# truemeat001/Simple-Raytracing-Render

Hardware: AMD Instinct MI355X
Metric: Msamples/s (rays x bounces) + HBM GB/s vs roofline, Cornell+teapot 1024spp (higher is better)
Workload: dtype f32

## Files before the change

simple-raytracing-render_amd/csrc/kernels.h:

```cpp
#pragma once
#include <hip/hip_runtime.h>

#include <cstdint>

#include "device_scene.h"

namespace srr {

struct SceneView {
  const DObj* objs;
  int n_world;
  int has_media;
  const DXform* xforms;
  const DSphere* spheres;
  const DRect* rects;
  const DStandaloneTri* stris;
  const DMesh* meshes;
  const float4* nodes;
  const float4* node4;
  int node4_lds;
  int node4_total;
  const float4* node4q;
  int node4_lds_q;
  int use_q;
// ... 60 lines not shown
  uint32_t l = 0;
  while ((1ull << l) < d) ++l;
  const uint32_t p = 31 + l;
  return UDiv31{(uint32_t)(((1ull << p) + d - 1) / d), p};
}

struct PathWork {
  const int32_t* pixels;
  const double* sobol;
  int npix, spp_w;
  int s_base;
  int nx, ny;
  UDiv31 div_spp, div_nx;
  uint64_t base_seed;
  int64_t n_paths;
  int max_depth;
  unsigned long long* cursor;
  unsigned long long* counters;
  float* sample;
  float* raw;
  uint8_t* rays;
  int keep_spp, keep_s0;
  float4* rec;
  int lanes;
  int* err;
  int stack_cap;
  int2* gstack;
  int gstack_cap;
  unsigned long long* wave_times;
  int deep_tries;
  float* slow_rays;
  unsigned* slow_count;
  int walk_q;
};

enum PathsCtr : int {
  kCtrWorldRays = 0,
  kCtrCursor = 1,
  kCtrError = 2,
  kCtrTicksRefill = 4,
  kCtrTicksWorld,
  kCtrTicksMesh,
  kCtrTicksShade,
  kCtrTicksFold,
  kCtrWaveIters = 9,
  kCtrTicksRecord = 10,
  kCtrStackOverflows = 11,
  kCtrDeepTraversals = 12,
  kCtrTicksMixture = 13,
  kCtrMixtureRounds = 14,
  kCtrMixtureCapped = 15,
  kCtrTicksBeck = 16, kCtrTicksSpec, kCtrTicksDiffSetup,
  kCtrItsBeck, kCtrItsSpec, kCtrItsDiff,
  kCtrLanesBeck, kCtrLanesSpec, kCtrLanesDiff,
  kCtrLanesInPath,
  kCtrMeshSteps, kCtrMeshLaneSteps, kCtrMeshWalkers,
  kCtrLeafTicks, kCtrLeafPasses,
  kCtrStepFetch, kCtrStepSlab, kCtrStepOrder,
  kCtrBeckAttempts,
  kCtrBeckAttemptsMax,
  kCtrSuspended = 36,
  kCtrTicksCamOnly = 37, kCtrItsCamOnly,
  kCtrTicksPretrace = 39, kCtrPretracePasses, kCtrShadeRounds,
  kPathsCtrCount
};
constexpr int kPathsCtrWords = 48;
static_assert(kPathsCtrCount == 42 && kPathsCtrCount <= kPathsCtrWords, "PathsCtr fits FrameSlot::ctr");
static_assert(kCtrTicksFold == kCtrTicksRefill + 4 && kCtrTicksFold < kCtrWaveIters, "phase ticks");
static_assert(kCtrTicksDiffSetup == kCtrTicksBeck + 2 && kCtrItsBeck == kCtrTicksBeck + 3 && kCtrItsDiff == kCtrItsBeck + 2 &&
                  kCtrLanesBeck == kCtrItsBeck + 3 && kCtrLanesDiff == kCtrLanesBeck + 2 && kCtrLanesInPath == 25,
              "family words");
static_assert(kCtrMeshSteps == 26 && kCtrStepOrder == kCtrStepFetch + 2 && kCtrBeckAttemptsMax == 35 &&
                  kCtrBeckAttemptsMax < kCtrSuspended, "mesh words");
static_assert(kCtrDeepTraversals == kCtrStackOverflows + 1, "TraceCtx::ovf counts overflows, ovf[1] deep traversals");
static_assert(kCtrItsCamOnly == 38 && kCtrShadeRounds == 41, "camera-only and pre-trace words");
#ifndef SRR_KSTACK
#define SRR_KSTACK 8
#endif
constexpr int kPathsLdsStack = SRR_KSTACK;
constexpr int kPathsGlobalStack = 56;

constexpr int kPathsWorldLdsBytes = 8192;
#ifndef SRR_LDS_NODES
#define SRR_LDS_NODES 96
#endif
constexpr int kPathsLdsNodes = SRR_LDS_NODES;

constexpr int kRingRayWords = 11;
constexpr int kRingHitWord = kRingRayWords;
constexpr int kRingWordsHit = kRingHitWord + 3;
constexpr int ring_words(bool pretrace) { return pretrace ? kRingWordsHit : kRingRayWords; }
static_assert(ring_words(false) == 11 && ring_words(true) == 14 && kRingHitWord + 2 < kRingWordsHit, "ring entry layout");

constexpr int kLdsPerCu = 160 * 1024;
constexpr int paths_lds_fixed(int bs, bool wl) {
  return (wl ? kPathsWorldLdsBytes : 16) + 8 * kPathsLdsStack * bs + bs;
}
constexpr int paths_lds_nodes_big(bool pretrace) {
  return (kLdsPerCu - paths_lds_fixed(1024, true) - 4 * ring_words(pretrace) * 1024) / 128;
}
// ... 118 lines not shown
```

simple-raytracing-render_amd/csrc/kernels.hip:

```cpp
#include <hip/hip_runtime.h>

#include <cfloat>
#include <algorithm>
#include <cstdint>
#include <cstdlib>
#include <cstring>

#include "device_scene.h"
#include "devmath.h"
#include "kernels.h"
#include "../../include/srr/merl.h"

namespace srr {
namespace dev {

SRR_D V3 sphere_center(const DSphere& s, float tm, bool moving) {
  V3 c0 = v3(s.c0[0], s.c0[1], s.c0[2]);
  if (!moving) return c0;
  V3 c1 = v3(s.c1[0], s.c1[1], s.c1[2]);
  return c0 + ((tm - s.t0) / (s.t1 - s.t0)) * (c1 - c0);
}

SRR_D bool sphere_hit(const DSphere& s, bool moving, const Ray& r, float tmin, float tmax, float& t) {
  V3 oc = r.o - sphere_center(s, r.tm, moving);
// ... 2562 lines not shown
  float tm;
  double sx, sy;
  sobol2_point((uint32_t)(W.s_base + (int)s), sx, sy);
  camera_ray(S, pix, W.s_base + s, sx, sy, W.nx, W.ny, W.base_seed, o, d, tm, rng, &W.div_nx);
  r = Ray{o, d, tm};
}

template <int BS>
SRR_D void ring_put(lds_ptr<float> e, const Ray& r, const Rng& rng) {
  e[0] = r.o.x;
  e[BS] = r.o.y;
  e[2 * BS] = r.o.z;
  e[3 * BS] = r.d.x;
  e[4 * BS] = r.d.y;
  e[5 * BS] = r.d.z;
  e[6 * BS] = r.tm;
  e[7 * BS] = __uint_as_float((uint32_t)rng.lcg);
  e[8 * BS] = __uint_as_float((uint32_t)(rng.lcg >> 32));
  e[9 * BS] = __uint_as_float((uint32_t)rng.pcg);
  e[10 * BS] = __uint_as_float((uint32_t)(rng.pcg >> 32));
}

template <int BS>
SRR_D void ring_get_ray(lds_ptr<const float> e, Ray& r) {
  r = Ray{v3(e[0], e[BS], e[2 * BS]), v3(e[3 * BS], e[4 * BS], e[5 * BS]), e[6 * BS]};
}
template <int BS>
SRR_D void ring_get(lds_ptr<const float> e, Ray& r, Rng& rng) {
  ring_get_ray<BS>(e, r);
  rng.lcg = (uint64_t)__float_as_uint(e[7 * BS]) | ((uint64_t)__float_as_uint(e[8 * BS]) << 32);
  rng.pcg = (uint64_t)__float_as_uint(e[9 * BS]) | ((uint64_t)__float_as_uint(e[10 * BS]) << 32);
}

constexpr int kNoHit = -2;
template <int BS>
SRR_D void ring_put_hit(lds_ptr<float> e, int obj, int prim, float t) {
  e[kRingHitWord * BS] = __int_as_float(obj);
  e[(kRingHitWord + 1) * BS] = __int_as_float(prim);
  e[(kRingHitWord + 2) * BS] = t;
}
template <int BS>
SRR_D WorldHit ring_get_hit(lds_ptr<const float> e) {
  return WorldHit{__float_as_int(e[kRingHitWord * BS]), __float_as_int(e[(kRingHitWord + 1) * BS]), e[(kRingHitWord + 2) * BS]};
}

template <int BS, bool HIT>
SRR_D void ring_fill(lds_ptr<float> ring, const SceneView& S, const PathWork& W, uint32_t nb, uint32_t n_paths) {
  const uint32_t gi = nb + (uint32_t)lane_id();
  if (gi < n_paths) {
    Ray gr;
    Rng grng;
    path_camera_ray(S, W, gi, gr, grng);
    ring_put<BS>(ring + lane_id(), gr, grng);
    if (HIT) ring_put_hit<BS>(ring + lane_id(), kNoHit, -1, 0.f);
  }
}

template <int BS, bool HIT>
SRR_D void ring_take(lds_ptr<const float> e, Ray& r, Rng& rng, WorldHit& w) {
  ring_get<BS>(e, r, rng);
  if (HIT) w = ring_get_hit<BS>(e);
}

struct PathsArgs {
  SceneView S;
  PathWork W;
};
#if defined(__HIP_DEVICE_COMPILE__)
template <class T>
using kptr = const __attribute__((address_space(4))) T*;
SRR_D kptr<PathsArgs> paths_args() {
  kptr<PathsArgs> p = (kptr<PathsArgs>)__builtin_amdgcn_kernarg_segment_ptr();
  asm volatile("" : "+s"(p));
  return p;
}
#else
SRR_D const PathsArgs* paths_args() { return nullptr; }
#endif

struct PoolRanks {
  uint32_t cnt;
  uint32_t rank;
  uint32_t avail;
};
SRR_D PoolRanks pool_ranks(uint64_t nm, uint32_t pool, uint32_t pool_end) {
  return PoolRanks{(uint32_t)__popcll(nm), (uint32_t)__popcll(nm & ((1ull << lane_id()) - 1)), pool_end - pool};
}
SRR_D uint32_t pool_arm(uint32_t nxt_lane0) {
  if (lane_id() == 0) nxt_lane0 = (uint32_t)atomicAdd(paths_args()->W.cursor, (unsigned long long)kPoolChunk);
  return nxt_lane0;
}

#ifdef SRR_SLOW_RAYS
SRR_D void slow_ray_record(const PathWork& W, int g, int depth, const Ray& r_in, uint64_t t_w0, int steps, const WorldHit& wh,
                           int slot) {
// ... 14 lines not shown
      e[13] = wh.t;
      e[14] = __int_as_float(slot);
      e[15] = __int_as_float((int)(t_w0 & 0x7fffffff));
    }
  }
}
#endif

constexpr int kTpWords = 8, kTfWords = kCtrBeckAttemptsMax - kCtrTicksBeck + 1, kTzWords = 2, kTptWords = 3;
constexpr int kTpPhases = kCtrTicksFold - kCtrTicksRefill + 1;
template <int Q>
constexpr int tp_at() {
  constexpr int at = Q >= kCtrTicksRefill && Q <= kCtrTicksFold ? Q - kCtrTicksRefill
                     : Q == kCtrTicksRecord ? kTpPhases : Q == kCtrTicksMixture ? kTpPhases + 1
                     : Q == kCtrMixtureRounds ? kTpPhases + 2 : -1;
  static_assert(at >= 0 && at < kTpWords, "not a word of tp");
  return at;
}
template <int Q>
constexpr int tf_at() {
  static_assert(Q >= kCtrTicksBeck && Q <= kCtrBeckAttemptsMax, "not a word of tf");
  return Q - kCtrTicksBeck;
}
template <int Q>
constexpr int tz_at() {
  static_assert(Q >= kCtrTicksCamOnly && Q < kCtrTicksCamOnly + kTzWords, "not a word of tz");
  return Q - kCtrTicksCamOnly;
}
template <int Q>
constexpr int tpt_at() {
  static_assert(Q >= kCtrTicksPretrace && Q < kCtrTicksPretrace + kTptWords, "not a word of tpt");
  return Q - kCtrTicksPretrace;
}

template <bool MEDIA, bool ALLFAM, int MINB, bool TIMED = false, bool WL = true, bool QUAD = false, bool CQ = false,
          int BS = kPathsBlock, bool SP = false>
#ifdef SRR_NUM_VGPR
#define SRR_PATHS_VGPR_ATTR __attribute__((amdgpu_num_vgpr(SRR_NUM_VGPR)))
#else
#define SRR_PATHS_VGPR_ATTR
#endif
__global__ void __launch_bounds__(BS, MINB) SRR_PATHS_VGPR_ATTR k_paths(PathsArgs A) {
  static_assert(BS == kPathsBlock || BS == 1024, "block size");
  (void)A;
  uint64_t tp[kTpWords] = {0, 0, 0, 0, 0, 0, 0, 0};
  uint64_t tf[kTfWords] = {0, 0, 0, 0, 0, 0, 0, 0, 0, 0, 0, 0, 0, 0, 0, 0, 0, 0, 0, 0};
  uint64_t tz[kTzWords] = {0, 0};
  uint64_t it = 0;
  uint64_t tpt[kTptWords] = {0, 0, 0};
  constexpr int TR = TR_BVH4_PRUNE | (WL ? TR_WL : 0) | (QUAD ? TR_QUAD : 0) | (CQ ? TR_Q : 0) | (BS == 1024 ? TR_BIG : 0) |
                     ((SP && !QUAD && !CQ) ? TR_SUSP : 0);
  __shared__ uint4 s_world[WL ? kWorldLdsBytes / 16 : 1];
  const auto view = [&]() {
    SceneView S = paths_args()->S;
    if constexpr (WL) {
      const char* b = (const char*)s_world;
      S.objs = (const DObj*)(b + S.world_off[0]);
      S.xforms = (const DXform*)(b + S.world_off[1]);
      S.spheres = (const DSphere*)(b + S.world_off[2]);
      S.rects = (const DRect*)(b + S.world_off[3]);
      S.stris = (const DStandaloneTri*)(b + S.world_off[4]);
      S.meshes = (const DMesh*)(b + S.world_off[5]);
      S.media = (const DMedium*)(b + S.world_off[6]);
      S.mats = (const DMat*)(b + S.world_off[7]);
      S.texs = (const DTex*)(b + S.world_off[8]);
      S.lights = (const DLight*)(b + S.world_off[9]);
// ... 18 lines not shown
  const uint32_t n_paths = (uint32_t)paths_args()->W.n_paths;
  const uint64_t t_start = paths_args()->W.wave_times ? __builtin_amdgcn_s_memrealtime() : 0;
  {
    const SceneView S0 = paths_args()->S;
    if constexpr (WL)
      for (int i = threadIdx.x; i < S0.world_words; i += blockDim.x) s_world[i] = S0.world_blob[i];
    const int n_lds_nodes = lds_nodes(S0);
    if (CQ)
      for (int i = threadIdx.x; i < n_lds_nodes * 4; i += blockDim.x) s_n4[i] = S0.node4q[i];
    else
      for (int i = threadIdx.x; i < n_lds_nodes * 8; i += blockDim.x) s_n4[i] = S0.node4[i];
  }
  __syncthreads();
  const int slot = blockIdx.x * blockDim.x + threadIdx.x;
  const auto rec_at = [&](const PathWork& W, int k) -> float4* {
    int s = slot;
    asm volatile("" : "+v"(s));
    return W.rec + ((size_t)k * W.lanes + s);
  };
  int g = -1;
  uint32_t pool = 0, pool_end = 0;
  uint32_t nxt_lane0 = 0;
  bool nxt_armed = false;
  uint32_t nxt_base = 0;
  bool nxt_ready = false;
  Ray r{};
  Rng rng{};
  int depth = 0;
  int walking = 0;
  uint32_t nrays = 0;
  uint32_t n_events = 0;
  constexpr uint32_t kCapped = 1, kSuspended = 1u << 12;
  uint32_t n_iter = 0, max_rounds = 0;
  WorldHit w{kNoHit, -1, 0};
  bool fill = false;
  for (;;) {
    ++n_iter;
    uint64_t tq = TIMED ? __builtin_amdgcn_s_memtime() : 0;
    if constexpr (!PT) {
    w = WorldHit{-1, -1, 0};
    const bool need = g < 0;
    const uint64_t nm = __ballot(need);
    if (nm && pool < n_paths) {
      const SceneView S = view();
      const PathWork W = work();
      const PoolRanks k = pool_ranks(nm, pool, pool_end);
      const uint32_t cnt = k.cnt, rank = k.rank, avail = k.avail;
      uint32_t idx = 0;
      if (RING) {
        if (need && rank < avail) {
          const uint32_t i0 = pool + rank;
          if (i0 < n_paths) {
            g = (int)i0;
            ring_take<BS, false>(ringw + (i0 - ring_base), r, rng, w);
            depth = 0;
          }
        }
        if (avail >= cnt) {
          pool += cnt;
        } else {
          uint32_t nb;
          if (nxt_armed) {
            nb = nxt_ready ? nxt_base : __builtin_amdgcn_readfirstlane(nxt_lane0);
            nxt_armed = false;
            nxt_ready = false;
          } else {
            uint32_t b = 0;
            if (lane_id() == 0) b = (uint32_t)atomicAdd(W.cursor, (unsigned long long)kPoolChunk);
            nb = __builtin_amdgcn_readfirstlane(b);
          }
          ring_fill<BS, false>(ringw, S, W, nb, n_paths);
          __builtin_amdgcn_fence(__ATOMIC_SEQ_CST, "wavefront");
          ring_base = nb;
          if (need && rank >= avail) {
            const uint32_t i1 = nb + (rank - avail);
            if (i1 < n_paths) {
              g = (int)i1;
              ring_take<BS, false>(ringw + (i1 - nb), r, rng, w);
              depth = 0;
            }
          }
          pool = nb + (cnt - avail);
          pool_end = nb + (uint32_t)kPoolChunk;
        }
      } else if (avail >= cnt) {
        idx = pool + rank;
        pool += cnt;
      } else {
        uint32_t nb;
        if (nxt_armed) {
          nb = nxt_ready ? nxt_base : __builtin_amdgcn_readfirstlane(nxt_lane0);
          nxt_armed = false;
          nxt_ready = false;
        } else {
          uint32_t b = 0;
          if (lane_id() == 0) b = (uint32_t)atomicAdd(W.cursor, (unsigned long long)kPoolChunk);
          nb = __builtin_amdgcn_readfirstlane(b);
        }
        idx = rank < avail ? pool + rank : nb + (rank - avail);
        pool = nb + (cnt - avail);
        pool_end = nb + (uint32_t)kPoolChunk;
      }
      if (!RING && need && idx < n_paths) {
        g = (int)idx;
        path_camera_ray(S, W, idx, r, rng);
        depth = 0;
      }
    }
    if (!nxt_armed && pool_end < n_paths) {
      nxt_lane0 = pool_arm(nxt_lane0);
      nxt_armed = true;
    }
    if (__ballot(g >= 0) == 0) break;
    if (TIMED) tf[tf_at<kCtrLanesInPath>()] += __popcll(__ballot(g >= 0));
    if (TIMED) {
      __builtin_amdgcn_s_waitcnt(0);
      const uint64_t t = __builtin_amdgcn_s_memtime();
      tp[tp_at<kCtrTicksRefill>()] += t - tq;
      tq = t;
      ++it;
    }
    }
    const bool fill_now = PT && fill;
    bool act = g >= 0 && (!PT || w.obj == kNoHit);
    Ray tr = r;
    if constexpr (PT) {
      if (fill_now) {
        act = ring_base + (uint32_t)lane_id() < n_paths && !walking;
        if (act) ring_get_ray<BS>(ringw + lane_id(), tr);
      }
      if (TIMED) {
        tf[tf_at<kCtrLanesInPath>()] += __popcll(__ballot(g >= 0));
        ++it;
      }
    }
    if (act) {
      const SceneView S = view();
      const PathWork W = work();
      TraceCtx cx{nullptr, to_lds(s_node + threadIdx.x), to_lds(s_t + threadIdx.x)};
      cx.lds_nodes = (const __attribute__((address_space(3))) f32x4*)to_lds(s_n4);
      cx.lds_count = lds_nodes(S);
      cx.st_cap = min(W.stack_cap, kStack);
      cx.ovf = W.counters + kCtrStackOverflows;
      cx.gst = W.gstack;
      cx.gst_cap = W.gstack ? W.gstack_cap : 0;
      cx.gst_stride = W.lanes;
      cx.slot = slot;
      if constexpr ((TR & TR_SUSP) != 0) {
        cx.walk_thr = vreg(fill_now ? 0 : (int)((__popcll(__ballot(true)) * (uint32_t)paths_args()->W.walk_q) >> 6));
        cx.resume = fill_now ? vreg(0) : walking;
        cx.susp = vreg(0);
      }
#ifdef SRR_SLOW_RAYS
      const uint64_t t_w0 = __builtin_amdgcn_s_memrealtime();
      cx.last_steps = 0;
      const Ray r_in = tr;
#endif
      const WorldHit wh =
          world_hit<MEDIA, TIMED ? (TR_BVH4_TIMED | (WL ? TR_WL : 0) | (SP ? TR_SUSP : 0)) : TR>(S, tr, rng, cx);
      if (fill_now) {
        ring_put_hit<BS>(ringw + lane_id(), wh.obj, wh.prim, wh.t);
      } else {
        w = wh;
        if constexpr ((TR & TR_SUSP) != 0) {
          walking = cx.susp;
          if (walking) {
            w.obj = PT ? kNoHit : -1;
            n_events += kSuspended;
          }
        }
      }
#ifdef SRR_SLOW_RAYS
      slow_ray_record(W, g, depth, r_in, t_w0, cx.last_steps, wh, slot);
#endif
      if (TIMED) {
        const uint64_t t = __builtin_amdgcn_s_memtime();
        if (fill_now) {
          tpt[tpt_at<kCtrTicksPretrace>()] += t - tq;
          ++tpt[tpt_at<kCtrPretracePasses>()];
        } else {
          if (__ballot(depth != 0) == 0) {
            tz[tz_at<kCtrTicksCamOnly>()] += t - tq;
            ++tz[tz_at<kCtrItsCamOnly>()];
          }
          tp[tp_at<kCtrTicksWorld>()] += t - tq - cx.mesh_cycles;
          tp[tp_at<kCtrTicksMesh>()] += cx.mesh_cycles;
          tf[tf_at<kCtrMeshSteps>()] += cx.mesh_steps;
          tf[tf_at<kCtrMeshLaneSteps>()] += cx.mesh_lane_steps;
          tf[tf_at<kCtrMeshWalkers>()] += cx.mesh_walkers;
          tf[tf_at<kCtrLeafTicks>()] += cx.leaf_cycles;
          tf[tf_at<kCtrLeafPasses>()] += cx.leaf_passes;
          tf[tf_at<kCtrStepFetch>()] += cx.step_parts[0];
          tf[tf_at<kCtrStepSlab>()] += cx.step_parts[1];
          tf[tf_at<kCtrStepOrder>()] += cx.step_parts[2];
        }
        tq = t;
      }
    }
    if constexpr (PT) {
      if (fill_now) {
        __builtin_amdgcn_fence(__ATOMIC_SEQ_CST, "wavefront");
        fill = false;
      }
    }
    if (nxt_armed && !nxt_ready) {
      nxt_base = __builtin_amdgcn_readfirstlane(nxt_lane0);
      nxt_ready = true;
    }
#pragma nounroll
    for (int round = 0; round < (PT ? 2 : 1); ++round) {
    if constexpr (PT) {
      if (TIMED) tq = __builtin_amdgcn_s_memtime();
      const bool need = g < 0;
      const uint64_t nm = __ballot(need);
      if (nm && pool < n_paths) {
        const PoolRanks k = pool_ranks(nm, pool, pool_end);
        const uint32_t cnt = k.cnt, rank = k.rank, avail = k.avail;
        if (need && rank < avail) {
          const uint32_t i0 = pool + rank;
          if (i0 < n_paths) {
            g = (int)i0;
            ring_take<BS, true>(ringw + (i0 - ring_base), r, rng, w);
            depth = 0;
          }
        }
        if (avail >= cnt) {
          pool += cnt;
        } else {
          const SceneView S = view();
          const PathWork W = work();
          uint32_t nb;
          if (nxt_armed) {
            nb = nxt_ready ? nxt_base : __builtin_amdgcn_readfirstlane(nxt_lane0);
            nxt_armed = false;
            nxt_ready = false;
          } else {
            uint32_t b = 0;
            if (lane_id() == 0) b = (uint32_t)atomicAdd(W.cursor, (unsigned long long)kPoolChunk);
            nb = __builtin_amdgcn_readfirstlane(b);
          }
          __builtin_amdgcn_fence(__ATOMIC_SEQ_CST, "wavefront");
          ring_fill<BS, true>(ringw, S, W, nb, n_paths);
          __builtin_amdgcn_fence(__ATOMIC_SEQ_CST, "wavefront");
          ring_base = nb;
          pool = nb;
          pool_end = nb + (uint32_t)kPoolChunk;
          fill = nb < n_paths;
        }
      }
      if (TIMED) {
        __builtin_amdgcn_s_waitcnt(0);
        const uint64_t t = __builtin_amdgcn_s_memtime();
        tp[tp_at<kCtrTicksRefill>()] += t - tq;
        tq = t;
      }
      if (fill) break;
    }
    const bool sh = g >= 0 && (!PT || w.obj != kNoHit);
    if constexpr (PT) {
      if (__ballot(sh) == 0) break;
      if (TIMED) ++tpt[tpt_at<kCtrShadeRounds>()];
    }
    bool done = sh && (PT || !walking);
    V3 C = v3(0.f);
    bool diff = false, pend = false;
    int natt = 0;
    uint64_t fam_dt[3] = {0, 0, 0};
    DiffSetup ds{};
    V3 d_atten = v3(0.f), d_n = v3(0.f), d_dir = v3(0.f);
    float d_pdf = 0;
    int d_tries = 0;
    bool d_dead = false;
    if (sh) {
      if (w.obj >= 0) {
        const SceneView S = view();
        const PathWork W = work();
        const HitRec h = world_record<TR>(S, r, w);
        const int kind = h.mat >= 0 ? S.mats[h.mat].kind : -1;
        if (TIMED) {
          __builtin_amdgcn_s_waitcnt(0);
          const uint64_t t = __builtin_amdgcn_s_memtime();
          tp[tp_at<kCtrTicksRecord>()] += t - tq;
          tq = t;
        }
        const int fam = family_of(h.mat, kind, depth, W.max_depth);
        if (TIMED) {
          const uint64_t mb = __ballot(fam == FAM_BECK), ms = __ballot(fam == FAM_SPEC),
                         md = __ballot(fam == FAM_DIFF && S.n_lights > 0);
          tf[tf_at<kCtrItsBeck>()] += mb != 0; tf[tf_at<kCtrItsSpec>()] += ms != 0; tf[tf_at<kCtrItsDiff>()] += md != 0;
          tf[tf_at<kCtrLanesBeck>()] += __popcll(mb); tf[tf_at<kCtrLanesSpec>()] += __popcll(ms); tf[tf_at<kCtrLanesDiff>()] += __popcll(md);
        }
        if (fam == FAM_TERM) {
          C = hit_emitted(S, h.mat, r.d, h.p, h.n, h.u, h.v);
        } else if ((!ALLFAM || fam == FAM_DIFF) && S.n_lights > 0) {
          const DMat M = S.mats[h.mat];
          d_atten = tex_value(S, M.tex, h.u, h.v, h.p);
          Bsdf f;
          f.kind = M.kind;
          f.n = h.n;
          f.uvw = onb_from_w(h.n);
          f.A = M.p[0];
          f.B = M.p[1];
          bsdf_prepare<false>(f, r.d);
          ds = diff_setup(f, h.p);
          d_dead = bsdf_dead(S, f, h.p);
          (void)drand(rng);
          d_n = h.n;
          diff = pend = true;
          done = false;
          if (TIMED) fam_dt[2] = __builtin_amdgcn_s_memtime() - tq;
        } else {
          const DMat M = S.mats[h.mat];
          float4 rec;
          bool sp;
          V3 nd;
          float nt;
          const uint64_t tb = TIMED ? __builtin_amdgcn_s_memtime() : 0;
          if (!ALLFAM || fam == FAM_DIFF) scatter<FAM_DIFF>(S, M, r.d, r.tm, h.p, h.n, h.u, h.v, rng, rec, sp, nd, nt);
          else if (fam == FAM_BECK) {
            scatter<FAM_BECK>(S, M, r.d, r.tm, h.p, h.n, h.u, h.v, rng, rec, sp, nd, nt, TIMED ? &natt : nullptr);
            if (TIMED) fam_dt[0] = __builtin_amdgcn_s_memtime() - tb;
          } else {
            scatter<FAM_SPEC>(S, M, r.d, r.tm, h.p, h.n, h.u, h.v, rng, rec, sp, nd, nt);
            if (TIMED) fam_dt[1] = __builtin_amdgcn_s_memtime() - tb;
          }
          if (depth >= W.max_depth || slot >= W.lanes) atomicOr(W.err, 2);
          else *rec_at(W, depth) = rec;
          if (!sp && S.n_lights > 0 && rec.w == 0) n_events += kCapped;
          r = Ray{h.p, nd, nt};
          ++depth;
          done = false;
        }
      }
    }
    if (TIMED) {
      int sum = natt, mx = natt;
      for (int o = 32; o > 0; o >>= 1) {
        sum += __shfl_xor(sum, o);
        mx = max(mx, __shfl_xor(mx, o));
      }
      tf[tf_at<kCtrBeckAttempts>()] += sum;
      tf[tf_at<kCtrBeckAttemptsMax>()] += mx;
      for (int q = 0; q < 3; ++q) {
        uint64_t m = fam_dt[q];
        for (int o = 32; o > 0; o >>= 1) m = max(m, (uint64_t)__shfl_xor((unsigned long long)m, o));
        tf[tf_at<kCtrTicksBeck>() + q] += m;
      }
    }
    if (__ballot(pend)) {
      const SceneView S = view();
      const uint64_t t_mix = TIMED ? __builtin_amdgcn_s_memtime() : 0;
      int rounds = skip_mixture(S, ds, d_dead, pend, d_tries, rng.lcg, d_dir, d_pdf, 1);
      if (__ballot(pend)) rounds += coop_mixture(S, ds, pend, d_tries, rng.lcg, d_dir, d_pdf, paths_args()->W.deep_tries);
      if (TIMED) {
        tp[tp_at<kCtrTicksMixture>()] += __builtin_amdgcn_s_memtime() - t_mix;
        tp[tp_at<kCtrMixtureRounds>()] += rounds;
      }
      max_rounds = max(max_rounds, (uint32_t)rounds);
    }
    if (diff) {
      const PathWork W = work();
      if (d_pdf == 0) n_events += kCapped;
      float c = dot(d_n, unit_vector(d_dir));
      if (c < 0) c = 0;
      const V3 as = d_atten * (c / kPi);
      if (depth >= W.max_depth || slot >= W.lanes) atomicOr(W.err, 2);
      else *rec_at(W, depth) = make_float4(as.x, as.y, as.z, d_pdf);
      r = Ray{ds.p, d_dir, r.tm};
      ++depth;
    }
    if (sh) {
      const PathWork W = work();
      if (PT) w.obj = kNoHit;
      if (TIMED) {
        const uint64_t t = __builtin_amdgcn_s_memtime();
        tp[tp_at<kCtrTicksShade>()] += t - tq;
        tq = t;
      }
      if (done && (g >= W.n_paths || depth > W.max_depth)) {
        atomicOr(W.err, 4);
        g = -1;
        done = false;
      }
      if (done) {
        int k = depth - 1;
        for (; k >= 0; k -= 4) {
          float4 a[4];
#pragma unroll
          for (int j = 0; j < 4; ++j) a[j] = k - j >= 0 ? rec_load(rec_at(W, k - j)) : make_float4(0, 0, 0, 0);
#pragma unroll
          for (int j = 0; j < 4; ++j) {
            if (k - j < 0) break;
            const V3 av = v3(a[j].x, a[j].y, a[j].z);
            if (__float_as_uint(a[j].w) == kSpecMark) C = av * C;
            else C = v3(0.f) + (av * C) / a[j].w;
          }
        }
        if (W.raw) {
          const size_t kq = (size_t)(g / W.spp_w) * W.keep_spp + W.keep_s0 + (size_t)(g % W.spp_w);
          W.raw[3 * kq] = C.x;
          W.raw[3 * kq + 1] = C.y;
          W.raw[3 * kq + 2] = C.z;
          W.rays[kq] = (uint8_t)(depth + 1);
        }
        if (!(C.x == C.x)) C.x = 0;
        if (!(C.y == C.y)) C.y = 0;
        if (!(C.z == C.z)) C.z = 0;
        nts(&W.sample[3 * (size_t)g], C.x);
        nts(&W.sample[3 * (size_t)g + 1], C.y);
        nts(&W.sample[3 * (size_t)g + 2], C.z);
        nrays += depth + 1;
        g = -1;
      }
      if (TIMED) tp[tp_at<kCtrTicksFold>()] += __builtin_amdgcn_s_memtime() - tq;
    }
    }
    if constexpr (PT) {
      if (!nxt_armed && pool_end < n_paths) {
        nxt_lane0 = pool_arm(nxt_lane0);
        nxt_armed = true;
      }
      if (!fill && pool >= n_paths && __ballot(g >= 0) == 0) break;
    }
  }
  const PathWork W = work();
  if (TIMED && lane_id() == 0) {
    for (int q = 0; q < kTpPhases; ++q) atomicAdd(W.counters + kCtrTicksRefill + q, (unsigned long long)tp[q]);
    atomicAdd(W.counters + kCtrWaveIters, (unsigned long long)it);
    atomicAdd(W.counters + kCtrTicksRecord, (unsigned long long)tp[tp_at<kCtrTicksRecord>()]);
    atomicAdd(W.counters + kCtrTicksMixture, (unsigned long long)tp[tp_at<kCtrTicksMixture>()]);
    atomicAdd(W.counters + kCtrMixtureRounds, (unsigned long long)tp[tp_at<kCtrMixtureRounds>()]);
    for (int q = 0; q < kTfWords; ++q) atomicAdd(W.counters + kCtrTicksBeck + q, (unsigned long long)tf[q]);
    for (int q = 0; q < kTzWords; ++q) atomicAdd(W.counters + kCtrTicksCamOnly + q, (unsigned long long)tz[q]);
    for (int q = 0; q < kTptWords; ++q) atomicAdd(W.counters + kCtrTicksPretrace + q, (unsigned long long)tpt[q]);
  }

  unsigned long long tot = nrays;
  for (int o = 32; o > 0; o >>= 1) tot += __shfl_xor(tot, o);
  if (lane_id() == 0 && tot) atomicAdd(W.counters + kCtrWorldRays, tot);
  if (__ballot(n_events != 0)) {
    unsigned long long cap = n_events & (kSuspended - 1), su = n_events / kSuspended;
    for (int o = 32; o > 0; o >>= 1) {
      cap += __shfl_xor(cap, o);
      su += __shfl_xor(su, o);
    }
    if (lane_id() == 0) {
      if (cap) atomicAdd(W.counters + kCtrMixtureCapped, cap);
      if (su) atomicAdd(W.counters + kCtrSuspended, su);
    }
  }
  if (W.wave_times && lane_id() == 0) {
    const size_t wv = (size_t)(blockIdx.x * blockDim.x + threadIdx.x) / 64;
    W.wave_times[4 * wv] = t_start;
    W.wave_times[4 * wv + 1] = __builtin_amdgcn_s_memrealtime();
    W.wave_times[4 * wv + 2] = tot;
    W.wave_times[4 * wv + 3] = n_iter | ((unsigned long long)max_rounds << 32);
  }
}

constexpr int kAccChunk = 16;
struct AccOut {
  float* out;
  int scale_ns;
};
SRR_D void acc_write(float* acc, AccOut o, size_t a, float cx, float cy, float cz) {
  acc[a] = cx;
  acc[a + 1] = cy;
// ... 1026 lines not shown
```

simple-raytracing-render_amd/csrc/renderer.cpp:

```cpp
#include "renderer.h"

#include "multi.h"

#include <algorithm>
#include <chrono>
#include <cstdlib>
#include <cstring>
#include <memory>
#include <thread>
#include <cstdio>

namespace srr {

constexpr int kVisitWords = 3 + 2 * 64;

#define RCHK(x)                                                        \
  do {                                                                 \
    hipError_t e_ = (x);                                               \
    if (e_ != hipSuccess) {                                            \
      err = std::string(#x) + ": " + hipGetErrorString(e_);            \
      return SRR_EIO;                                                  \
    }                                                                  \
  } while (0)

// ... 311 lines not shown
  RCHK(hipEventCreate(&F.ev_end));
  RCHK(hipMalloc((void**)&F.ctr, kPathsCtrWords * sizeof(unsigned long long)));
  RCHK(hipHostMalloc((void**)&F.ctr_host, kPathsCtrWords * sizeof(unsigned long long)));
  return 0;
}

void slot_free(FrameSlot& F) {
  (void)hipFree(F.rec);
  (void)hipFree(F.gstack);
  (void)hipFree(F.sample);
  (void)hipFree(F.ctr);
  (void)hipFree(F.acc);
  if (F.ctr_host) (void)hipHostFree(F.ctr_host);
  for (hipEvent_t e : F.win_ev) (void)hipEventDestroy(e);
  if (F.ev_beg) (void)hipEventDestroy(F.ev_beg);
  if (F.ev_end) (void)hipEventDestroy(F.ev_end);
  if (F.own_stream && F.st) (void)hipStreamDestroy(F.st);
  F = FrameSlot{};
}

static void release_window(FrameSlot& F) {
  if (!F.sample) return;
  (void)hipFree(F.sample);
  F.sample = nullptr;
  F.sample_cap = 0;
}

struct PathsSetup {
  int gst_cap = 0;
  int walk_q = 0;
  int deep_tries = 32;
  int stack_cap = kPathsLdsStack;
  size_t budget = 0;
};

static int paths_prepare(srr_renderer* r, FrameSlot& F, int max_depth, PathsSetup& ps, std::string& err) {
  if (!r->pw_lanes) r->pw_lanes = paths_lanes_per_device(r->view, r->device);
  const size_t rec_need = (size_t)r->pw_lanes * std::max(1, max_depth);
  if (rec_need > F.rec_cap) {
    (void)hipFree(F.rec);
    F.rec = nullptr;
    F.rec_cap = 0;
    RCHK(hipMalloc((void**)&F.rec, rec_need * sizeof(float4)));
    F.rec_cap = rec_need;
  }
  const char* gs_env = getenv("SRR_GSTACK");
  ps.gst_cap = (r->has_meshes && !(gs_env && !atoi(gs_env))) ? kPathsGlobalStack : 0;
  if (ps.gst_cap && !F.gstack)
    RCHK(hipMalloc((void**)&F.gstack, (size_t)ps.gst_cap * r->pw_lanes * sizeof(int2) + 3 * (size_t)r->pw_lanes * sizeof(float4)));
  const char* wq_env = getenv("SRR_WALK_Q");
  ps.walk_q = wq_env ? std::max(0, std::min(64, atoi(wq_env))) : r->walk_q_default;
  ps.budget = (size_t)16384 << 20;
  if (const char* e = getenv("SRR_WINDOW_MB")) ps.budget = (size_t)std::max(1, atoi(e)) << 20;
  ps.budget /= (size_t)std::max(1, r->window_share);
  const char* dt_env = getenv("SRR_DEEP_TRIES");
  ps.deep_tries = dt_env ? std::max(0, atoi(dt_env)) : 32;
  ps.stack_cap = kPathsLdsStack;
  if (const char* e = getenv("SRR_STACK_CAP")) ps.stack_cap = std::max(1, std::min(kPathsLdsStack, atoi(e)));
  return 0;
}

static int window_samples(const PathsSetup& ps, int64_t npix, int spp) {
  const int64_t w_max = std::max<int64_t>(1, (((int64_t)1 << 31) - 1) / std::max<int64_t>(1, npix));
  int W = (int)std::max<int64_t>(
      1, std::min<int64_t>(std::min<int64_t>(spp, w_max), (int64_t)(ps.budget / (12 * (size_t)npix))));
  if (W < spp && W >= 16) W &= ~3;
  return W;
}

static int ensure_window(srr_renderer* r, FrameSlot& F, size_t win_paths, std::string& err) {
  if (win_paths > F.sample_cap) {
    (void)hipFree(F.sample);
    F.sample = nullptr;
    F.sample_cap = 0;
    hipError_t e = hipMalloc((void**)&F.sample, win_paths * 3 * sizeof(float));
    if (e == hipErrorOutOfMemory) {
      (void)hipGetLastError();
      if (&F == &r->sync_slot) {
        drain_async(r);
        for (FrameSlot& A : r->async_slots) release_window(A);
      } else {
        release_window(r->sync_slot);
      }
      e = hipMalloc((void**)&F.sample, win_paths * 3 * sizeof(float));
    }
    RCHK(e);
    F.sample_cap = win_paths;
  }
  return 0;
}

static PathWork paths_work(srr_renderer* r, FrameSlot& F, const srr_params* p, const PathsSetup& ps,
                           const int32_t* pixels, int64_t npix, int s_first, int Wn) {
  PathWork w{};
  w.pixels = pixels;
  w.sobol = r->sobol + 2 * (size_t)s_first;
  w.npix = (int)npix;
  w.spp_w = Wn;
  w.s_base = s_first;
  w.nx = p->nx;
  w.ny = p->ny;
  w.div_spp = make_udiv31((uint32_t)Wn);
  w.div_nx = make_udiv31((uint32_t)p->nx);
  w.base_seed = p->base_seed;
  w.n_paths = (int64_t)npix * Wn;
  w.max_depth = p->max_depth;
  w.cursor = F.ctr + kCtrCursor;
  w.counters = F.ctr;
  w.sample = F.sample;
  w.rec = F.rec;
  w.err = (int*)(F.ctr + kCtrError);
  const int64_t bl = paths_block_lanes(r->view);
  w.lanes = (int)std::min<int64_t>(r->pw_lanes, ((w.n_paths + bl - 1) / bl) * bl);
  w.stack_cap = ps.stack_cap;
  w.gstack = ps.gst_cap ? F.gstack : nullptr;
  w.gstack_cap = ps.gst_cap;
  w.deep_tries = ps.deep_tries;
  w.walk_q = ps.gst_cap ? ps.walk_q : 0;
  return w;
}

static int paths_enqueue(srr_renderer* r, FrameSlot& F, const srr_params* p, bool identity, int64_t npix,
                         float* acc, bool zero_pending, int64_t acc_total, float* d_mean, bool diagnostics,
                         std::string& err) {
  const bool keep = (p->flags & SRR_FLAG_KEEP_PATHS) != 0;
  hipStream_t st = F.st;
  PathsSetup ps;
  {
    const int rc = paths_prepare(r, F, p->max_depth, ps, err);
    if (rc < 0) return rc;
  }
  const int W = window_samples(ps, npix, p->spp);
  if ((int64_t)npix * W >= ((int64_t)1 << 31)) {
    err = "frame too large for one sample window (npix >= 2^31)";
    return SRR_EINVAL;
  }
  {
    const int rc = ensure_window(r, F, (size_t)npix * W, err);
    if (rc < 0) return rc;
  }
  RCHK(hipMemsetAsync(F.ctr, 0, kPathsCtrWords * sizeof(unsigned long long), st));
  const bool want_sums = (p->flags & SRR_FLAG_SUMS) != 0;
  const int n_windows = (p->spp + W - 1) / W;
  while ((int)F.win_ev.size() < 2 * n_windows) {
    hipEvent_t e;
    RCHK(hipEventCreate(&e));
    F.win_ev.push_back(e);
  }
  F.n_windows = n_windows;
  const bool all_fam = !r->diffuse_only;
  static const bool want_wave_times = getenv("SRR_WAVE_TIMES") != nullptr;
// ... 88 lines not shown
  if (getenv("SRR_PATHS_TIMING") && ctr[kCtrWaveIters]) {
    const double it = (double)ctr[kCtrWaveIters];
    fprintf(stderr, "k_paths per wave-iteration (ticks): refill %.0f  world %.0f  mesh %.0f  record %.0f  scatter %.0f  fold %.0f  (%llu wave-iterations)\n",
            ctr[kCtrTicksRefill] / it, ctr[kCtrTicksWorld] / it, ctr[kCtrTicksMesh] / it, ctr[kCtrTicksRecord] / it,
            (ctr[kCtrTicksShade] - ctr[kCtrTicksRecord]) / it, ctr[kCtrTicksFold] / it, ctr[kCtrWaveIters]);
    fprintf(stderr, "  scatter: mixture loop %.0f ticks, %.2f rounds per wave-iteration\n", ctr[kCtrTicksMixture] / it,
            ctr[kCtrMixtureRounds] / it);
    auto per = [](unsigned long long a, unsigned long long b) { return b ? (double)a / (double)b : 0.0; };
    fprintf(stderr, "  families: beck %.0f ticks/it (runs in %.1f %% of its, %.1f lanes/run), spec %.0f (%.1f %%, %.1f), "
                    "diff set-up %.0f (%.1f %%, %.1f); lanes in a path %.1f of 64\n",
            ctr[kCtrTicksBeck] / it, 100 * ctr[kCtrItsBeck] / it, per(ctr[kCtrLanesBeck], ctr[kCtrItsBeck]),
            ctr[kCtrTicksSpec] / it, 100 * ctr[kCtrItsSpec] / it, per(ctr[kCtrLanesSpec], ctr[kCtrItsSpec]),
            ctr[kCtrTicksDiffSetup] / it, 100 * ctr[kCtrItsDiff] / it, per(ctr[kCtrLanesDiff], ctr[kCtrItsDiff]),
            ctr[kCtrLanesInPath] / it);
    fprintf(stderr, "  mesh: longest walk %.1f node steps/it, %.1f lane steps/it over %.1f walking lanes, "
                    "%.0f ticks per step of the longest walk\n",
            ctr[kCtrMeshSteps] / it, ctr[kCtrMeshLaneSteps] / it, ctr[kCtrMeshWalkers] / it,
            per(ctr[kCtrTicksMesh], ctr[kCtrMeshSteps]));
    fprintf(stderr, "  mesh leaf queue: %.0f ticks/it, %.1f passes/it (%.0f ticks per pass)\n", ctr[kCtrLeafTicks] / it,
            ctr[kCtrLeafPasses] / it, per(ctr[kCtrLeafTicks], ctr[kCtrLeafPasses]));
    fprintf(stderr, "  mesh step parts (ticks/it): node fetch %.0f  slab + queue %.0f  order + push + pop %.0f\n",
            ctr[kCtrStepFetch] / it, ctr[kCtrStepSlab] / it, ctr[kCtrStepOrder] / it);
    fprintf(stderr, "  beckmann mixture: %.2f attempts per Beckmann scatter, %.2f for the wave's slowest lane per run\n",
            per(ctr[kCtrBeckAttempts], ctr[kCtrLanesBeck]), per(ctr[kCtrBeckAttemptsMax], ctr[kCtrItsBeck]));
    fprintf(stderr, "  suspended walks: %.2f lanes per wave-iteration\n", ctr[kCtrSuspended] / it);
    fprintf(stderr, "  camera-ray-only iterations (every tracing lane at depth 0): %llu of %llu, world + mesh %.0f ticks "
                    "per wave-iteration of them; the others %.0f\n",
            ctr[kCtrItsCamOnly], ctr[kCtrWaveIters], per(ctr[kCtrTicksCamOnly], ctr[kCtrItsCamOnly]),
            per(ctr[kCtrTicksWorld] + ctr[kCtrTicksMesh] - ctr[kCtrTicksCamOnly], ctr[kCtrWaveIters] - ctr[kCtrItsCamOnly]));
    fprintf(stderr, "  pre-trace: %llu passes of the %llu wave-iterations, %.0f ticks each (%.0f per wave-iteration); "
                    "shade rounds %.2f per wave-iteration\n",
            ctr[kCtrPretracePasses], ctr[kCtrWaveIters], per(ctr[kCtrTicksPretrace], ctr[kCtrPretracePasses]),
            ctr[kCtrTicksPretrace] / it, ctr[kCtrShadeRounds] / it);
  }
#ifdef SRR_SLOW_RAYS
  if (r->pw_slow) {
    unsigned n = 0;
    RCHK(hipMemcpy(&n, r->pw_slow + 16 * 65536, sizeof(unsigned), hipMemcpyDeviceToHost));
    n = std::min(n, 65536u);
    std::vector<float> v(16 * (size_t)n);
    if (n) RCHK(hipMemcpy(v.data(), r->pw_slow, v.size() * sizeof(float), hipMemcpyDeviceToHost));
    auto I = [&](size_t k) { int x; memcpy(&x, &v[k], 4); return x; };
    for (unsigned i = 0; i < n; ++i) {
      const size_t b = 16 * (size_t)i;
      fprintf(stderr, "SLOWRAY {\"g\": %d, \"depth\": %d, \"o\": [%.9g, %.9g, %.9g], \"d\": [%.9g, %.9g, %.9g], "
              "\"tm\": %.9g, \"ticks\": %d, \"steps\": %d, \"obj\": %d, \"prim\": %d, \"t\": %.9g, \"slot\": %d, "
              "\"t0\": %d, \"spp_w\": %d}\n", I(b), I(b + 1), v[b + 2], v[b + 3], v[b + 4], v[b + 5], v[b + 6], v[b + 7], v[b + 8],
              I(b + 9), I(b + 10), I(b + 11), I(b + 12), v[b + 13], I(b + 14), I(b + 15), p->spp);
    }
  }
#else
  (void)r;
  (void)p;
#endif
  if (ctr[kCtrError]) {
    err = "k_paths index guard tripped (bits " + std::to_string(ctr[kCtrError]) + ")";
    return SRR_EIO;
  }
  float total = 0;
  RCHK(hipEventElapsedTime(&total, F.ev_beg, F.ev_end));
  s.world_rays = (int64_t)ctr[kCtrWorldRays];
  s.stack_overflows = (int64_t)ctr[kCtrStackOverflows];
  s.deep_traversals = (int64_t)ctr[kCtrDeepTraversals];
  s.mixture_capped = (int64_t)ctr[kCtrMixtureCapped];
  s.walks_suspended = (int64_t)ctr[kCtrSuspended];
  s.paths = F.paths;
// ... 706 lines not shown
```

Baseline: 9328.

## Replace pre-trace ring refill with head/tail wave scheduling and LDS path pool

Restructures the persistent path-tracing loop for the diffuse-only (PT) kernel. A wave now launches a full chunk of camera paths together (head), and once live lanes drop to a threshold it compacts the survivors into an LDS pool, together with their throughput records copied from a separate head record area. Tail passes then resume pooled paths until the pool is small enough to start a new head chunk. This replaces the previous scheme of pre-tracing refill rays and running two shade rounds per iteration, and is meant to cut divergence and idle lanes. It doubles the record buffer size and adds compaction and copy overhead.

```diff
diff --git a/simple-raytracing-render_amd/csrc/kernels.h b/simple-raytracing-render_amd/csrc/kernels.h
--- a/simple-raytracing-render_amd/csrc/kernels.h
+++ b/simple-raytracing-render_amd/csrc/kernels.h
@@ -116,7 +116,9 @@
   float* slow_rays;
   unsigned* slow_count;
   int walk_q;
-};
+  int tail_min, pool_cap;
+};
+constexpr int kPathsTailMin = 48;
 
 enum PathsCtr : int {
   kCtrWorldRays = 0,
@@ -146,10 +148,13 @@
   kCtrSuspended = 36,
   kCtrTicksCamOnly = 37, kCtrItsCamOnly,
   kCtrTicksPretrace = 39, kCtrPretracePasses, kCtrShadeRounds,
+  kCtrTicksHead = 42, kCtrHeadPasses, kCtrHeadLanes,
+  kCtrTicksTail, kCtrTailPasses, kCtrTailLanes,
   kPathsCtrCount
 };
 constexpr int kPathsCtrWords = 48;
-static_assert(kPathsCtrCount == 42 && kPathsCtrCount <= kPathsCtrWords, "PathsCtr fits FrameSlot::ctr");
+static_assert(kPathsCtrCount == 48 && kPathsCtrCount <= kPathsCtrWords, "PathsCtr fits FrameSlot::ctr");
+static_assert(kCtrTailLanes == kCtrTicksHead + 5, "head and tail words");
 static_assert(kCtrTicksFold == kCtrTicksRefill + 4 && kCtrTicksFold < kCtrWaveIters, "phase ticks");
 static_assert(kCtrTicksDiffSetup == kCtrTicksBeck + 2 && kCtrItsBeck == kCtrTicksBeck + 3 && kCtrItsDiff == kCtrItsBeck + 2 &&
                   kCtrLanesBeck == kCtrItsBeck + 3 && kCtrLanesDiff == kCtrLanesBeck + 2 && kCtrLanesInPath == 25,
diff --git a/simple-raytracing-render_amd/csrc/kernels.hip b/simple-raytracing-render_amd/csrc/kernels.hip
--- a/simple-raytracing-render_amd/csrc/kernels.hip
+++ b/simple-raytracing-render_amd/csrc/kernels.hip
@@ -2618,19 +2618,29 @@
   rng.pcg = (uint64_t)__float_as_uint(e[9 * BS]) | ((uint64_t)__float_as_uint(e[10 * BS]) << 32);
 }
 
-constexpr int kNoHit = -2;
 template <int BS>
-SRR_D void ring_put_hit(lds_ptr<float> e, int obj, int prim, float t) {
-  e[kRingHitWord * BS] = __int_as_float(obj);
-  e[(kRingHitWord + 1) * BS] = __int_as_float(prim);
-  e[(kRingHitWord + 2) * BS] = t;
+SRR_D void pool_put(lds_ptr<float> e, const Ray& r, const Rng& rng, int g, int depth) {
+  e[0] = r.o.x;
+  e[BS] = r.o.y;
+  e[2 * BS] = r.o.z;
+  e[3 * BS] = r.d.x;
+  e[4 * BS] = r.d.y;
+  e[5 * BS] = r.d.z;
+  e[6 * BS] = r.tm;
+  e[7 * BS] = __uint_as_float((uint32_t)rng.lcg);
+  e[8 * BS] = __uint_as_float((uint32_t)(rng.lcg >> 32));
+  e[9 * BS] = __int_as_float(g);
+  e[10 * BS] = __int_as_float(depth);
 }
 template <int BS>
-SRR_D WorldHit ring_get_hit(lds_ptr<const float> e) {
-  return WorldHit{__float_as_int(e[kRingHitWord * BS]), __float_as_int(e[(kRingHitWord + 1) * BS]), e[(kRingHitWord + 2) * BS]};
-}
-
-template <int BS, bool HIT>
+SRR_D void pool_get(lds_ptr<const float> e, Ray& r, Rng& rng, int& g, int& depth) {
+  ring_get_ray<BS>(e, r);
+  rng.lcg = (uint64_t)__float_as_uint(e[7 * BS]) | ((uint64_t)__float_as_uint(e[8 * BS]) << 32);
+  g = __float_as_int(e[9 * BS]);
+  depth = __float_as_int(e[10 * BS]);
+}
+
+template <int BS>
 SRR_D void ring_fill(lds_ptr<float> ring, const SceneView& S, const PathWork& W, uint32_t nb, uint32_t n_paths) {
   const uint32_t gi = nb + (uint32_t)lane_id();
   if (gi < n_paths) {
@@ -2638,15 +2648,9 @@
     Rng grng;
     path_camera_ray(S, W, gi, gr, grng);
     ring_put<BS>(ring + lane_id(), gr, grng);
-    if (HIT) ring_put_hit<BS>(ring + lane_id(), kNoHit, -1, 0.f);
-  }
-}
-
-template <int BS, bool HIT>
-SRR_D void ring_take(lds_ptr<const float> e, Ray& r, Rng& rng, WorldHit& w) {
-  ring_get<BS>(e, r, rng);
-  if (HIT) w = ring_get_hit<BS>(e);
-}
+  }
+}
+
 
 struct PathsArgs {
   SceneView S;
@@ -2727,6 +2731,8 @@
   static_assert(Q >= kCtrTicksPretrace && Q < kCtrTicksPretrace + kTptWords, "not a word of tpt");
   return Q - kCtrTicksPretrace;
 }
+constexpr int kThtWords = kCtrTailLanes - kCtrTicksHead + 1;
+constexpr int kHeadLiveMin = 32;
 
 template <bool MEDIA, bool ALLFAM, int MINB, bool TIMED = false, bool WL = true, bool QUAD = false, bool CQ = false,
           int BS = kPathsBlock, bool SP = false>
@@ -2811,11 +2817,70 @@
   uint32_t n_events = 0;
   constexpr uint32_t kCapped = 1, kSuspended = 1u << 12;
   uint32_t n_iter = 0, max_rounds = 0;
-  WorldHit w{kNoHit, -1, 0};
-  bool fill = false;
+  WorldHit w{-1, -1, 0};
+  uint64_t used = 0;
+  uint64_t walkm = 0;
+  bool head = false, tail = false;
+  int passes = 0;
+  uint32_t last_end = 0;
+  uint64_t tht[kThtWords] = {0, 0, 0, 0, 0, 0};
+  const auto rec_row = [&](const PathWork& W, int k) { return PT && !tail ? k + W.max_depth : k; };
   for (;;) {
     ++n_iter;
     uint64_t tq = TIMED ? __builtin_amdgcn_s_memtime() : 0;
+    const uint64_t t_pass = tq;
+    if constexpr (PT) {
+      if (!head) {
+        const PathWork W = work();
+        if (last_end < n_paths && walkm == 0 && __popcll(used) < max(1, W.tail_min)) {
+          uint32_t nb;
+          if (nxt_armed) {
+            nb = nxt_ready ? nxt_base : __builtin_amdgcn_readfirstlane(nxt_lane0);
+            nxt_armed = false;
+            nxt_ready = false;
+          } else {
+            uint32_t b = 0;
+            if (lane_id() == 0) b = (uint32_t)atomicAdd(W.cursor, (unsigned long long)kPoolChunk);
+            nb = __builtin_amdgcn_readfirstlane(b);
+          }
+          last_end = nb + (uint32_t)kPoolChunk;
+          if (nb < n_paths) {
+            const SceneView S = view();
+            const uint32_t gi = nb + (uint32_t)lane_id();
+            if (gi < n_paths) {
+              path_camera_ray(S, W, gi, r, rng);
+              g = (int)gi;
+              depth = 0;
+            }
+            head = true;
+            passes = 0;
+          }
+        }
+        if (!head) {
+          if (used == 0) break;
+          tail = true;
+          if ((used >> lane_id()) & 1) {
+            pool_get<BS>(ringw + lane_id(), r, rng, g, depth);
+            if constexpr (SP) walking = (int)((walkm >> lane_id()) & 1);
+          }
+        }
+      }
+      if (!nxt_armed && last_end < n_paths) {
+        nxt_lane0 = pool_arm(nxt_lane0);
+        nxt_armed = true;
+      }
+      if (TIMED) {
+        __builtin_amdgcn_s_waitcnt(0);
+        const uint64_t t = __builtin_amdgcn_s_memtime();
+        tp[tp_at<kCtrTicksRefill>()] += t - tq;
+        tq = t;
+        const int n_in = __popcll(__ballot(g >= 0));
+        tf[tf_at<kCtrLanesInPath>()] += n_in;
+        ++it;
+        ++tht[tail ? kCtrTailPasses - kCtrTicksHead : kCtrHeadPasses - kCtrTicksHead];
+        tht[tail ? kCtrTailLanes - kCtrTicksHead : kCtrHeadLanes - kCtrTicksHead] += n_in;
+      }
+    }
     if constexpr (!PT) {
     w = WorldHit{-1, -1, 0};
     const bool need = g < 0;
@@ -2831,7 +2896,7 @@
           const uint32_t i0 = pool + rank;
           if (i0 < n_paths) {
             g = (int)i0;
-            ring_take<BS, false>(ringw + (i0 - ring_base), r, rng, w);
+            ring_get<BS>(ringw + (i0 - ring_base), r, rng);
             depth = 0;
           }
         }
@@ -2848,14 +2913,14 @@
             if (lane_id() == 0) b = (uint32_t)atomicAdd(W.cursor, (unsigned long long)kPoolChunk);
             nb = __builtin_amdgcn_readfirstlane(b);
           }
-          ring_fill<BS, false>(ringw, S, W, nb, n_paths);
+          ring_fill<BS>(ringw, S, W, nb, n_paths);
           __builtin_amdgcn_fence(__ATOMIC_SEQ_CST, "wavefront");
           ring_base = nb;
           if (need && rank >= avail) {
             const uint32_t i1 = nb + (rank - avail);
             if (i1 < n_paths) {
               g = (int)i1;
-              ring_take<BS, false>(ringw + (i1 - nb), r, rng, w);
+              ring_get<BS>(ringw + (i1 - nb), r, rng);
               depth = 0;
             }
           }
@@ -2900,19 +2965,9 @@
       ++it;
     }
     }
-    const bool fill_now = PT && fill;
-    bool act = g >= 0 && (!PT || w.obj == kNoHit);
-    Ray tr = r;
-    if constexpr (PT) {
-      if (fill_now) {
-        act = ring_base + (uint32_t)lane_id() < n_paths && !walking;
-        if (act) ring_get_ray<BS>(ringw + lane_id(), tr);
-      }
-      if (TIMED) {
-        tf[tf_at<kCtrLanesInPath>()] += __popcll(__ballot(g >= 0));
-        ++it;
-      }
-    }
+    const bool head_now = PT && !tail;
+    const bool act = g >= 0;
+    const Ray tr = r;
     if (act) {
       const SceneView S = view();
       const PathWork W = work();
@@ -2926,8 +2981,8 @@
       cx.gst_stride = W.lanes;
       cx.slot = slot;
       if constexpr ((TR & TR_SUSP) != 0) {
-        cx.walk_thr = vreg(fill_now ? 0 : (int)((__popcll(__ballot(true)) * (uint32_t)paths_args()->W.walk_q) >> 6));
-        cx.resume = fill_now ? vreg(0) : walking;
+        cx.walk_thr = vreg(head_now ? 0 : (int)((__popcll(__ballot(true)) * (uint32_t)paths_args()->W.walk_q) >> 6));
+        cx.resume = walking;
         cx.susp = vreg(0);
       }
 #ifdef SRR_SLOW_RAYS
@@ -2937,16 +2992,12 @@
 #endif
       const WorldHit wh =
           world_hit<MEDIA, TIMED ? (TR_BVH4_TIMED | (WL ? TR_WL : 0) | (SP ? TR_SUSP : 0)) : TR>(S, tr, rng, cx);
-      if (fill_now) {
-        ring_put_hit<BS>(ringw + lane_id(), wh.obj, wh.prim, wh.t);
-      } else {
-        w = wh;
-        if constexpr ((TR & TR_SUSP) != 0) {
-          walking = cx.susp;
-          if (walking) {
-            w.obj = PT ? kNoHit : -1;
-            n_events += kSuspended;
-          }
+      w = wh;
+      if constexpr ((TR & TR_SUSP) != 0) {
+        walking = cx.susp;
+        if (walking) {
+          w.obj = -1;
+          n_events += kSuspended;
         }
       }
 #ifdef SRR_SLOW_RAYS
@@ -2954,7 +3005,7 @@
 #endif
       if (TIMED) {
         const uint64_t t = __builtin_amdgcn_s_memtime();
-        if (fill_now) {
+        if (head_now && passes == 0) {
           tpt[tpt_at<kCtrTicksPretrace>()] += t - tq;
           ++tpt[tpt_at<kCtrPretracePasses>()];
         } else {
@@ -2976,71 +3027,14 @@
         tq = t;
       }
     }
-    if constexpr (PT) {
-      if (fill_now) {
-        __builtin_amdgcn_fence(__ATOMIC_SEQ_CST, "wavefront");
-        fill = false;
-      }
-    }
     if (nxt_armed && !nxt_ready) {
       nxt_base = __builtin_amdgcn_readfirstlane(nxt_lane0);
       nxt_ready = true;
     }
-#pragma nounroll
-    for (int round = 0; round < (PT ? 2 : 1); ++round) {
-    if constexpr (PT) {
-      if (TIMED) tq = __builtin_amdgcn_s_memtime();
-      const bool need = g < 0;
-      const uint64_t nm = __ballot(need);
-      if (nm && pool < n_paths) {
-        const PoolRanks k = pool_ranks(nm, pool, pool_end);
-        const uint32_t cnt = k.cnt, rank = k.rank, avail = k.avail;
-        if (need && rank < avail) {
-          const uint32_t i0 = pool + rank;
-          if (i0 < n_paths) {
-            g = (int)i0;
-            ring_take<BS, true>(ringw + (i0 - ring_base), r, rng, w);
-            depth = 0;
-          }
-        }
-        if (avail >= cnt) {
-          pool += cnt;
-        } else {
-          const SceneView S = view();
-          const PathWork W = work();
-          uint32_t nb;
-          if (nxt_armed) {
-            nb = nxt_ready ? nxt_base : __builtin_amdgcn_readfirstlane(nxt_lane0);
-            nxt_armed = false;
-            nxt_ready = false;
-          } else {
-            uint32_t b = 0;
-            if (lane_id() == 0) b = (uint32_t)atomicAdd(W.cursor, (unsigned long long)kPoolChunk);
-            nb = __builtin_amdgcn_readfirstlane(b);
-          }
-          __builtin_amdgcn_fence(__ATOMIC_SEQ_CST, "wavefront");
-          ring_fill<BS, true>(ringw, S, W, nb, n_paths);
-          __builtin_amdgcn_fence(__ATOMIC_SEQ_CST, "wavefront");
-          ring_base = nb;
-          pool = nb;
-          pool_end = nb + (uint32_t)kPoolChunk;
-          fill = nb < n_paths;
-        }
-      }
-      if (TIMED) {
-        __builtin_amdgcn_s_waitcnt(0);
-        const uint64_t t = __builtin_amdgcn_s_memtime();
-        tp[tp_at<kCtrTicksRefill>()] += t - tq;
-        tq = t;
-      }
-      if (fill) break;
-    }
-    const bool sh = g >= 0 && (!PT || w.obj != kNoHit);
-    if constexpr (PT) {
-      if (__ballot(sh) == 0) break;
-      if (TIMED) ++tpt[tpt_at<kCtrShadeRounds>()];
-    }
-    bool done = sh && (PT || !walking);
+    {
+    const bool sh = g >= 0 && !(PT && walking);
+    if (PT && TIMED) ++tpt[tpt_at<kCtrShadeRounds>()];
+    bool done = sh && !walking;
     V3 C = v3(0.f);
     bool diff = false, pend = false;
     int natt = 0;
@@ -3104,7 +3098,7 @@
             if (TIMED) fam_dt[1] = __builtin_amdgcn_s_memtime() - tb;
           }
           if (depth >= W.max_depth || slot >= W.lanes) atomicOr(W.err, 2);
-          else *rec_at(W, depth) = rec;
+          else *rec_at(W, rec_row(W, depth)) = rec;
           if (!sp && S.n_lights > 0 && rec.w == 0) n_events += kCapped;
           r = Ray{h.p, nd, nt};
           ++depth;
@@ -3144,13 +3138,12 @@
       if (c < 0) c = 0;
       const V3 as = d_atten * (c / kPi);
       if (depth >= W.max_depth || slot >= W.lanes) atomicOr(W.err, 2);
-      else *rec_at(W, depth) = make_float4(as.x, as.y, as.z, d_pdf);
+      else *rec_at(W, rec_row(W, depth)) = make_float4(as.x, as.y, as.z, d_pdf);
       r = Ray{ds.p, d_dir, r.tm};
       ++depth;
     }
     if (sh) {
       const PathWork W = work();
-      if (PT) w.obj = kNoHit;
       if (TIMED) {
         const uint64_t t = __builtin_amdgcn_s_memtime();
         tp[tp_at<kCtrTicksShade>()] += t - tq;
@@ -3166,7 +3159,7 @@
         for (; k >= 0; k -= 4) {
           float4 a[4];
 #pragma unroll
-          for (int j = 0; j < 4; ++j) a[j] = k - j >= 0 ? rec_load(rec_at(W, k - j)) : make_float4(0, 0, 0, 0);
+          for (int j = 0; j < 4; ++j) a[j] = k - j >= 0 ? rec_load(rec_at(W, rec_row(W, k - j))) : make_float4(0, 0, 0, 0);
 #pragma unroll
           for (int j = 0; j < 4; ++j) {
             if (k - j < 0) break;
@@ -3195,11 +3188,44 @@
     }
     }
     if constexpr (PT) {
-      if (!nxt_armed && pool_end < n_paths) {
-        nxt_lane0 = pool_arm(nxt_lane0);
-        nxt_armed = true;
-      }
-      if (!fill && pool >= n_paths && __ballot(g >= 0) == 0) break;
+      const uint64_t live = __ballot(g >= 0);
+      if (tail) {
+        if (g >= 0) pool_put<BS>(ringw + lane_id(), r, rng, g, depth);
+        used = live;
+        if constexpr (SP) walkm = __ballot(g >= 0 && walking != 0);
+        g = -1;
+        walking = 0;
+        __builtin_amdgcn_fence(__ATOMIC_SEQ_CST, "wavefront");
+      } else {
+        ++passes;
+        const PathWork W = work();
+        const int n_live = __popcll(live);
+        const uint64_t fr0 = (W.pool_cap >= 64 ? ~0ull : (1ull << max(1, W.pool_cap)) - 1) & ~used;
+        if (live == 0) {
+          head = false;
+        } else if (passes >= 2 && n_live <= kHeadLiveMin && n_live <= (int)__popcll(fr0)) {
+          int s = 0;
+          uint64_t lv = live, fr = fr0;
+          while (lv) {
+            if (lane_id() == __ffsll((unsigned long long)lv) - 1) s = __ffsll((unsigned long long)fr) - 1;
+            lv &= lv - 1;
+            fr &= fr - 1;
+          }
+          if (g >= 0) {
+            pool_put<BS>(ringw + s, r, rng, g, depth);
+            const int col = slot - lane_id() + s;
+            if (depth > W.max_depth || slot >= W.lanes) atomicOr(W.err, 2);
+            else
+              for (int j = 0; j < depth; ++j) W.rec[(size_t)j * W.lanes + col] = *rec_at(W, j + W.max_depth);
+          }
+          used |= fr0 & ~fr;
+          g = -1;
+          head = false;
+          __builtin_amdgcn_fence(__ATOMIC_SEQ_CST, "workgroup");
+        }
+      }
+      if (TIMED) tht[tail ? kCtrTicksTail - kCtrTicksHead : 0] += __builtin_amdgcn_s_memtime() - t_pass;
+      tail = false;
     }
   }
   const PathWork W = work();
@@ -3212,6 +3238,8 @@
     for (int q = 0; q < kTfWords; ++q) atomicAdd(W.counters + kCtrTicksBeck + q, (unsigned long long)tf[q]);
     for (int q = 0; q < kTzWords; ++q) atomicAdd(W.counters + kCtrTicksCamOnly + q, (unsigned long long)tz[q]);
     for (int q = 0; q < kTptWords; ++q) atomicAdd(W.counters + kCtrTicksPretrace + q, (unsigned long long)tpt[q]);
+    if (PT)
+      for (int q = 0; q < kThtWords; ++q) atomicAdd(W.counters + kCtrTicksHead + q, (unsigned long long)tht[q]);
   }
 
   unsigned long long tot = nrays;
diff --git a/simple-raytracing-render_amd/csrc/renderer.cpp b/simple-raytracing-render_amd/csrc/renderer.cpp
--- a/simple-raytracing-render_amd/csrc/renderer.cpp
+++ b/simple-raytracing-render_amd/csrc/renderer.cpp
@@ -367,11 +367,14 @@
   int deep_tries = 32;
   int stack_cap = kPathsLdsStack;
   size_t budget = 0;
+  int tail_min = kPathsTailMin;
+  int pool_cap = 64;
 };
 
 static int paths_prepare(srr_renderer* r, FrameSlot& F, int max_depth, PathsSetup& ps, std::string& err) {
   if (!r->pw_lanes) r->pw_lanes = paths_lanes_per_device(r->view, r->device);
-  const size_t rec_need = (size_t)r->pw_lanes * std::max(1, max_depth);
+  const bool head_cols = r->diffuse_only && !r->view.has_media;
+  const size_t rec_need = (head_cols ? 2 : 1) * (size_t)r->pw_lanes * std::max(1, max_depth);
   if (rec_need > F.rec_cap) {
     (void)hipFree(F.rec);
     F.rec = nullptr;
@@ -390,6 +393,8 @@
   ps.budget /= (size_t)std::max(1, r->window_share);
   const char* dt_env = getenv("SRR_DEEP_TRIES");
   ps.deep_tries = dt_env ? std::max(0, atoi(dt_env)) : 32;
+  if (const char* e = getenv("SRR_TAIL_MIN")) ps.tail_min = std::max(1, std::min(64, atoi(e)));
+  if (const char* e = getenv("SRR_POOL_CAP")) ps.pool_cap = std::max(1, std::min(64, atoi(e)));
   ps.stack_cap = kPathsLdsStack;
   if (const char* e = getenv("SRR_STACK_CAP")) ps.stack_cap = std::max(1, std::min(kPathsLdsStack, atoi(e)));
   return 0;
@@ -452,6 +457,8 @@
   w.gstack_cap = ps.gst_cap;
   w.deep_tries = ps.deep_tries;
   w.walk_q = ps.gst_cap ? ps.walk_q : 0;
+  w.tail_min = ps.tail_min;
+  w.pool_cap = ps.pool_cap;
   return w;
 }
 
@@ -606,6 +613,9 @@
                     "shade rounds %.2f per wave-iteration\n",
             ctr[kCtrPretracePasses], ctr[kCtrWaveIters], per(ctr[kCtrTicksPretrace], ctr[kCtrPretracePasses]),
             ctr[kCtrTicksPretrace] / it, ctr[kCtrShadeRounds] / it);
+    fprintf(stderr, "  head passes: %llu, %.0f ticks each, %.1f lanes in a path; tail passes: %llu, %.0f ticks each, %.1f lanes\n",
+            ctr[kCtrHeadPasses], per(ctr[kCtrTicksHead], ctr[kCtrHeadPasses]), per(ctr[kCtrHeadLanes], ctr[kCtrHeadPasses]),
+            ctr[kCtrTailPasses], per(ctr[kCtrTicksTail], ctr[kCtrTailPasses]), per(ctr[kCtrTailLanes], ctr[kCtrTailPasses]));
   }
 #ifdef SRR_SLOW_RAYS
   if (r->pw_slow) {
```

Result: faster. 9908 (median of 6 runs) (+6.2%).
